# Digital-Defiance/node-fhe-accelerate

Hardware: AMD Instinct MI355X
Metric: NTTs/s at degree 16384 (batched, forward NTT + pointwise modmul) (higher is better)
Workload: dtype u64 (32-bit Shoup/Montgomery lanes for q<2^30); 1 GPU; C3: N=16384 forward NTT + modmul, batch 65536 per GPU, q=132120577; n=16384, batch_per_gpu=65536, global_batch=65536, q=132120577, parallelism=batch-sharded x1, no data-path collective

## Files before the change

node-fhe-accelerate_amd/csrc/fhe_gpu.cpp:

```cpp
#include <hip/hip_runtime.h>

#include <algorithm>
#include <cstdlib>
#include <cstdio>
#include <cstring>
#include <mutex>
#include <thread>
#include <string>
#include <vector>

#include "../../include/fhe_gpu.h"
#include "fhe_internal.hpp"
#include "keygen.hpp"
#include "build_id.h"

using u64 = uint64_t;
using u32 = uint32_t;
using u128 = unsigned __int128;

namespace {

thread_local std::string g_err;

int fail(int code, const std::string &msg) {
// ... 816 lines not shown
        c->inv_n = ref_mod_inverse(n, q);
    }
    c->fwd_tw.resize(n);
    c->inv_tw.resize(n);
    c->fwd_tw[0] = c->inv_tw[0] = 1;
    for (u32 i = 1; i < n; ++i) {
        c->fwd_tw[i] = mulmod(c->fwd_tw[i - 1], psi, q);
        c->inv_tw[i] = mulmod(c->inv_tw[i - 1], c->psi_inv, q);
    }
    DeviceGuard g(device);
    int rc = c->word == 32 ? build_tables<u32>(c, c->plan.a32) : build_tables<u64>(c, c->plan.a64);
    if (rc == FHE_OK && c->wide) rc = build_wide_tables(c);
    if (rc == FHE_OK && (int)logn > FHE_NS::kMaxFusedLogN) {
        c->plan.big_chunk = ((size_t)1 << 25) >> logn;
        for (auto &sp : c->plan.big_scratch) {
            hipError_t e = hipMalloc((void **)&sp, c->plan.big_chunk * n * sizeof(u64));
            if (e != hipSuccess) { rc = hip_fail(e, "hipMalloc(big-N scratch)"); break; }
        }
    }
    if (rc == FHE_OK) {
        hipError_t e = hipStreamCreateWithFlags(&c->own_stream, hipStreamNonBlocking);
        if (e != hipSuccess) rc = hip_fail(e, "hipStreamCreate");
    }
    if (rc == FHE_OK) {
        const char *kv = std::getenv("FHE_POOL_KEEP_MB");
        const uint64_t keep_mb = kv ? std::strtoull(kv, nullptr, 10) : 8192;
        hipMemPool_t pool = nullptr;
        if (keep_mb && hipDeviceGetDefaultMemPool(&pool, device) == hipSuccess && pool) {
            uint64_t keep = keep_mb << 20;
            (void)hipMemPoolSetAttribute(pool, hipMemPoolAttrReleaseThreshold, &keep);
        }
        (void)hipGetLastError();
    }
    if (rc != FHE_OK) {
        free_tables(c);
        delete c;
        return rc;
    }
    c->stream = c->own_stream;
    c->plan.logn = logn;
    c->plan.word = c->word;
    {
        int cus = 0;
        if (hipDeviceGetAttribute(&cus, hipDeviceAttributeMultiprocessorCount, device) != hipSuccess || cus <= 0) cus = 256;
        (void)hipGetLastError();
        c->plan.cus = cus;
    }
    c->plan.wide = c->wide;
    c->plan.lazy = c->word == 32 && (u128)(4 + 2 * logn) * q <= ((u128)1 << 32);
    {
        const char *u = std::getenv("FHE_UNIT_TW");
        c->plan.compat = c->mode == FHE_MODE_COMPAT && !(u && u[0] == '0');
    }
    c->plan.stream = c->stream;
    c->plan.big_sync = &c->big_sync;
    *out = c;
    return FHE_OK;
}

int fhe_ctx_create_multi(uint32_t n, uint64_t q, int mode, const int *devices, int ndev, fhe_ctx **out) {
    if (!out) return fail(FHE_ERR_INVALID_ARG, "null out");
    *out = nullptr;
    if (!devices || ndev < 1) return fail(FHE_ERR_INVALID_ARG, "at least one device required");
    fhe_ctx *m = new fhe_ctx();
    for (int i = 0; i < ndev; ++i) {
        fhe_ctx *s = nullptr;
        const int rc = fhe_ctx_create(n, q, mode, devices[i], &s);
        if (rc != FHE_OK) {
            const std::string msg = g_err;
            fhe_ctx_destroy(m);
            return fail(rc, msg);
        }
        m->subs.push_back(s);
    }
    const fhe_ctx *s0 = m->subs[0];
    m->n = s0->n; m->logn = s0->logn; m->q = s0->q; m->psi = s0->psi; m->psi_inv = s0->psi_inv;
    m->inv_n = s0->inv_n; m->mode = s0->mode; m->device = s0->device; m->word = s0->word;
    m->fwd_tw = s0->fwd_tw; m->inv_tw = s0->inv_tw;
    m->stream = s0->stream;
    *out = m;
    return FHE_OK;
}

int fhe_ctx_device_count(const fhe_ctx *c, int *ndev) {
    if (int rc = check_ctx(c)) return rc;
    if (!ndev) return fail(FHE_ERR_INVALID_ARG, "null out");
    *ndev = c->multi() ? (int)c->subs.size() : 1;
    return FHE_OK;
}

int fhe_ctx_sub(const fhe_ctx *c, int i, fhe_ctx **out) {
    if (int rc = check_ctx(c)) return rc;
    if (!out) return fail(FHE_ERR_INVALID_ARG, "null out");
    const int nd = c->multi() ? (int)c->subs.size() : 1;
    if (i < 0 || i >= nd) return fail(FHE_ERR_INVALID_ARG, "device index out of range");
    *out = c->multi() ? c->subs[i] : const_cast<fhe_ctx *>(c);
    return FHE_OK;
}

void fhe_ctx_destroy(fhe_ctx *c) {
    if (!c) return;
    if (c->multi()) {
        for (auto it = c->subs.rbegin(); it != c->subs.rend(); ++it) fhe_ctx_destroy(*it);
        delete c;
        return;
    }
// ... 2291 lines not shown
```

node-fhe-accelerate_amd/csrc/fhe_internal.hpp:

```cpp
#pragma once
#include <hip/hip_runtime.h>
#include <stddef.h>
#include <stdint.h>

#include <mutex>

#include "ntt_core.hpp"

namespace FHE_NS {

struct BigSync {
    std::mutex mu;
    hipEvent_t done = nullptr;
    hipStream_t last = nullptr;
};

struct WideArgs {
    const uint64_t *twf, *twi;
    uint64_t q, qinv, mu;
    uint64_t r2;
    uint64_t ninv_m;
    uint64_t ninv_r2;
};

struct Plan {
    uint32_t logn;
    int word;
    int wide;
    int lazy;
    int compat;
    int cus;
    hipStream_t stream;
    uint64_t *big_scratch[2];
    size_t big_chunk;
    BigSync *big_sync;
    NttArgs<uint32_t> a32;
    NttArgs<uint64_t> a64;
    WideArgs wa;
};

constexpr int kMinLogN = 2;
constexpr int kMaxFusedLogN = 14;
constexpr int kMaxLogN = 16;

hipError_t launch_fwd(const Plan &p, const uint64_t *in, uint64_t *out, size_t batch, int epi);
hipError_t launch_inv(const Plan &p, const uint64_t *in, uint64_t *out, size_t batch);
hipError_t launch_fwd_mul(const Plan &p, const uint64_t *a, const uint64_t *w, uint64_t *out, size_t batch);
hipError_t launch_polymul(const Plan &p, const uint64_t *a, const uint64_t *b, uint64_t *c, size_t batch);
hipError_t launch_fwd_limbs(const Plan &p, const void *tab, int limbs, const uint64_t *in, uint64_t *out,
                            size_t batch);
hipError_t launch_inv_limbs(const Plan &p, const void *tab, int limbs, const uint64_t *a, const uint64_t *b,
                            uint64_t *c, size_t batch);
hipError_t launch_wide(const Plan &p, int op, const uint64_t *a, const uint64_t *b, uint64_t *c, size_t batch);
hipError_t launch_big(const Plan &p, int op, const uint64_t *a, const uint64_t *b, uint64_t *c, size_t batch);
hipError_t launch_extprod(const Plan &p, int k1, int level, int base_log, const uint64_t *glwe,
                          const uint64_t *ggsw, uint64_t *out, size_t batch);
bool extprod_acc_supported(const Plan &p, int k1, int level, int base_log);
hipError_t launch_extprod_acc(const Plan &p, int level, int base_log, const uint64_t *glwe, const uint64_t *ggsw,
                              uint64_t *out, size_t batch);

hipError_t launch_relin(const Plan &p, int level, int base_log, const uint64_t *ct3, const uint64_t *rlk,
                        uint64_t *out, size_t batch);
hipError_t launch_cmux_rotate(const Plan &p, int k1, int level, int base_log, const uint64_t *acc_in,
                              const uint64_t *ggsw, uint64_t *acc_out, size_t batch, const uint64_t *lwe_a,
                              uint32_t lwe_dim, uint32_t step, uint64_t lwe_q);
bool br_persist_supported(const Plan &p, int k1);
struct BrPairOpts {
    uint64_t timeout_ticks;
    bool coop;
    unsigned long long *repairs;
    bool multi;
};
bool br_pair_supported(const Plan &p, int k1, size_t batch);
int br_multi_members(const Plan &p, int level, size_t batch);
size_t br_pair_scratch_bytes(const Plan &p, size_t batch, int level, bool multi);
hipError_t launch_br_pair(const Plan &p, int level, int base_log, uint64_t *acc, const uint64_t *bsk,
                          const uint64_t *lwe_a, const uint64_t *lwe_b, uint32_t lwe_dim, uint64_t lwe_q, size_t batch,
                          void *scratch, const BrPairOpts &o);
hipError_t launch_br_persist(const Plan &p, int k1, int level, int base_log, uint64_t *acc, const uint64_t *bsk,
                             const uint64_t *lwe_a, const uint64_t *lwe_b, uint32_t lwe_dim, uint64_t lwe_q,
                             size_t batch);
hipError_t launch_cmux(const Plan &p, int k1, int level, int base_log, const uint64_t *ggsw, const uint64_t *ct0,
                       const uint64_t *ct1, uint64_t *out, size_t batch);
hipError_t launch_ct_mul(const Plan &p, const uint64_t *x, const uint64_t *y, uint64_t *out, size_t batch);
// ... 110 lines not shown
```

node-fhe-accelerate_amd/csrc/ntt_core.hpp:

```cpp
#pragma once
#include "fhe_arith.hpp"

namespace FHE_NS {

constexpr int kPadA[17] = {0, 0, 0, 0, 0, 3, 3, 3, 4, 5, 5, 6, 7, 8, 5, 5, 0};
constexpr int kPadB[17] = {0, 0, 0, 0, 0, 0, 0, 0, 0, 0, 0, 0, 0, 0, 10, 10, 0};

constexpr int gk(int logn, int loge) { return logn | (loge << 8); }
constexpr int gk_logn(int k) { return k & 0xff; }
constexpr int gk_loge(int k) { return ((k >> 8) & 0xf) ? ((k >> 8) & 0xf) : ((k & 0xff) < 4 ? (k & 0xff) : 4); }
constexpr int gk_sparse(int k, int sel) { return k | (sel << 12); }
constexpr int gk_sp(int k) { return (k >> 12) & 3; }
constexpr int gk_compat(int k) { return k | (1 << 14); }
constexpr bool gk_cp(int k) { return (k >> 14) & 1; }

constexpr int pad_a(int L, int E) {
    return E == 5 ? 0 : (L == 10 && E == 3) ? 5 : (L == 10 && E == 2) ? 4 : kPadA[L];
}
constexpr int pad_b(int L, int E) {
    return E == 5 ? L - 5 : (L == 10 && E == 3) ? 6 : (L == 10 && E == 2) ? 5 : kPadB[L];
}
template <int K>
__host__ __device__ constexpr uint32_t pad_idx(uint32_t i) {
    constexpr int L = gk_logn(K);
// ... 286 lines not shown
}

struct NoHook {
    __device__ void operator()() const {}
};

template <int LOGN, int PASS, int K, int LOOK, bool LAZY, typename W>
__device__ __forceinline__ void fwd_stages(uint32_t tau, W (&v)[Geo<LOGN>::E], Tw<W> (&t)[PassTw<LOGN, PASS>::COUNT],
                                           const Tw<W> *__restrict__ tw, const Arith<W> &ar) {
    constexpr int R = PassTw<LOGN, PASS>::R;
    if constexpr (K < R) {
        if constexpr (K + LOOK < R) load_tw<LOGN, PASS, W, K + LOOK, K + LOOK + 1>(tau, tw, t);
        fwd_stage<LOGN, PASS, K, LAZY>(v, t, ar);
        __builtin_amdgcn_sched_barrier(0);
        fwd_stages<LOGN, PASS, K + 1, LOOK, LAZY>(tau, v, t, tw, ar);
    }
}
template <int LOGN, int PASS, int K, int LOOK, bool FOLD, typename W>
__device__ __forceinline__ void inv_stages(uint32_t tau, W (&v)[Geo<LOGN>::E], Tw<W> (&t)[PassTw<LOGN, PASS>::COUNT],
                                           const Tw<W> *__restrict__ tw, const Arith<W> &ar, Scale<W> scale) {
    if constexpr (K >= 0) {
        if constexpr (K - LOOK >= 0) load_tw<LOGN, PASS, W, K - LOOK, K - LOOK + 1>(tau, tw, t);
        inv_stage<LOGN, PASS, K, FOLD>(v, t, ar, scale);
        __builtin_amdgcn_sched_barrier(0);
        inv_stages<LOGN, PASS, K - 1, LOOK, FOLD>(tau, v, t, tw, ar, scale);
    }
}
template <int LOGN>
constexpr bool staged_tw() { return Geo<LOGN>::LOGE >= 5; }

#ifndef FHE_STREAM_DEPTH
#define FHE_STREAM_DEPTH 4
#endif
template <int LOGN, typename W>
constexpr bool stream_tw() { return sizeof(W) == 8 && Geo<LOGN>::LOGE == 5; }
#ifndef FHE_STREAM_TW2
#define FHE_STREAM_TW2 0
#endif
template <int LOGN, typename W>
constexpr bool stream_tw2() { return FHE_STREAM_TW2 && Geo<LOGN>::LOGE == 5; }
constexpr int kStreamDepth = FHE_STREAM_DEPTH;

struct SItem { int k, u, tl; };
__host__ __device__ constexpr SItem stream_item(int R, int NU, bool inv, int i) {
    for (int s = 0; s < R; ++s) {
        const int k = inv ? R - 1 - s : s;
        if (i < NU << k) return SItem{k, i >> k, i & ((1 << k) - 1)};
        i -= NU << k;
    }
    return SItem{0, 0, 0};
}

template <int LOGN, int PASS, typename W>
__device__ __forceinline__ Tw<W> tw_one(uint32_t tau, const Tw<W> *__restrict__ tw, SItem it) {
    using G = Geo<LOGN>;
    constexpr int S = G::S(PASS);
    if constexpr (PASS == 0) {
        typedef const __attribute__((address_space(4))) W cw_t;
        const cw_t *cp = (const cw_t *)(const void *)tw;
        const uint32_t idx = (1u << it.k) + uint32_t(it.tl);
        return Tw<W>{cp[2 * idx], cp[2 * idx + 1]};
    } else {
        static_assert(G::P == 1, "streamed twiddles: one polynomial per workgroup");
        constexpr uint32_t m = (1u << S) - 1;
        const uint32_t cst = (1u << (S + it.k)) + ((uint32_t(it.u) << G::LOGT) & m) + (uint32_t(it.tl) << S);
        return bload_tw<W>(brsrc(tw), (tau & m) * (uint32_t)sizeof(Tw<W>), cst * (uint32_t)sizeof(Tw<W>));
    }
}

template <int LOGN, int PASS, bool INV, bool SKIP0, int I, typename W>
__device__ __forceinline__ void stream_load(uint32_t tau, const Tw<W> *__restrict__ tw,
                                            Tw<W> (&b)[PassTw<LOGN, PASS>::COUNT]) {
    using P = PassTw<LOGN, PASS>;
    if constexpr (I < P::COUNT) {
        constexpr SItem it = stream_item(P::R, P::NU, INV, I);
        if constexpr (!(SKIP0 && it.k == 0))
            b[I] = tw_one<LOGN, PASS>(tau, tw, it);
    }
}
template <int LOGN, int PASS, bool INV, bool SKIP0, int I = 0, typename W>
__device__ __forceinline__ void stream_begin(uint32_t tau, const Tw<W> *__restrict__ tw,
                                             Tw<W> (&b)[PassTw<LOGN, PASS>::COUNT]) {
    if constexpr (I < kStreamDepth) {
        stream_load<LOGN, PASS, INV, SKIP0, I>(tau, tw, b);
        stream_begin<LOGN, PASS, INV, SKIP0, I + 1>(tau, tw, b);
    }
}
template <int LOGN, int PASS, bool LAZY, bool RS, bool D2 = false, int I = 0, typename W>
__device__ __forceinline__ void fwd_pass_stream(uint32_t tau, W (&v)[Geo<LOGN>::E], Tw<W> (&b)[PassTw<LOGN, PASS>::COUNT],
                                                const Tw<W> *__restrict__ tw, const Arith<W> &ar, Scale<W> rmod = Scale<W>{},
                                                W (*v2)[Geo<LOGN>::E] = nullptr) {
    using P = PassTw<LOGN, PASS>;
    constexpr int R = P::R;
    constexpr bool SK = RS && PASS == 0;
    if constexpr (I < P::COUNT) {
        stream_load<LOGN, PASS, false, SK, I + kStreamDepth>(tau, tw, b);
        constexpr SItem it = stream_item(R, P::NU, false, I);
        constexpr int k = it.k;
#pragma unroll
        for (int h = 0; h < (D2 ? 2 : 1); ++h) {
            W (&x)[Geo<LOGN>::E] = h ? *v2 : v;
#pragma unroll
            for (int tt = 0; tt < (1 << R); ++tt) {
                if ((tt & (1 << k)) || (tt & ((1 << k) - 1)) != it.tl) continue;
                const int e = tt + (it.u << R), e2 = e + (1 << k);
                if constexpr (SK && k == 0) ar.template ct_rscale<gk_sp(LOGN)>(x[e], x[e2], rmod);
                else if constexpr (LAZY) ar.template ct_lazy<gk_sp(LOGN)>(x[e], x[e2], b[I]);
                else ar.template ct<gk_sp(LOGN)>(x[e], x[e2], b[I]);
            }
        }
        __builtin_amdgcn_sched_barrier(0);
        fwd_pass_stream<LOGN, PASS, LAZY, RS, D2, I + 1>(tau, v, b, tw, ar, rmod, v2);
    }
}
template <int LOGN, int PASS, bool FOLD, bool D2 = false, int I = 0, typename W>
__device__ __forceinline__ void inv_pass_stream(uint32_t tau, W (&v)[Geo<LOGN>::E], Tw<W> (&b)[PassTw<LOGN, PASS>::COUNT],
                                                const Tw<W> *__restrict__ tw, const Arith<W> &ar, Scale<W> scale,
                                                W (*v2)[Geo<LOGN>::E] = nullptr) {
    using P = PassTw<LOGN, PASS>;
    constexpr int R = P::R;
    constexpr bool SK = FOLD && PASS == 0;
    if constexpr (I < P::COUNT) {
        stream_load<LOGN, PASS, true, SK, I + kStreamDepth>(tau, tw, b);
        constexpr SItem it = stream_item(R, P::NU, true, I);
        constexpr int k = it.k;
#pragma unroll
        for (int h = 0; h < (D2 ? 2 : 1); ++h) {
            W (&x)[Geo<LOGN>::E] = h ? *v2 : v;
#pragma unroll
            for (int tt = 0; tt < (1 << R); ++tt) {
                if ((tt & (1 << k)) || (tt & ((1 << k) - 1)) != it.tl) continue;
                const int e = tt + (it.u << R), e2 = e + (1 << k);
                if constexpr (SK && k == 0) ar.template gs_scaled<gk_sp(LOGN)>(x[e], x[e2], scale);
                else ar.template gs<gk_sp(LOGN)>(x[e], x[e2], b[I]);
            }
        }
        __builtin_amdgcn_sched_barrier(0);
        inv_pass_stream<LOGN, PASS, FOLD, D2, I + 1>(tau, v, b, tw, ar, scale, v2);
    }
}

template <int LOGN, int PASS, bool LAZY, int PF, typename W, typename H = NoHook>
__device__ __forceinline__ void fwd_rest(W *lds, W (&v)[Geo<LOGN>::E], uint32_t tau, const Tw<W> *__restrict__ tw,
                                         const Arith<W> &ar, H &&hook = NoHook{}) {
    using G = Geo<LOGN>;
    if constexpr (PASS < G::NP) {
        Tw<W> t[PassTw<LOGN, PASS>::COUNT];
        if constexpr (stream_tw<LOGN, W>()) {
            stream_begin<LOGN, PASS, false, false>(tau, tw, t);
            exchange<LOGN, PASS - 1, PASS>(lds, v, tau);
            if constexpr (PASS == G::NP - 1) hook();
            fwd_pass_stream<LOGN, PASS, LAZY, false>(tau, v, t, tw, ar);
            fwd_rest<LOGN, PASS + 1, LAZY, PF>(lds, v, tau, tw, ar, hook);
            return;
        }
        load_tw<LOGN, PASS, W, 0, PF>(tau, tw, t);
        exchange<LOGN, PASS - 1, PASS>(lds, v, tau);
        if constexpr (staged_tw<LOGN>()) {
            if constexpr (PASS == G::NP - 1) hook();
            fwd_stages<LOGN, PASS, 0, PF, LAZY>(tau, v, t, tw, ar);
        } else {
            load_tw<LOGN, PASS, W, PF, 8>(tau, tw, t);
            if constexpr (PASS == G::NP - 1) hook();
            fwd_pass<LOGN, PASS, LAZY>(v, t, ar);
        }
        fwd_rest<LOGN, PASS + 1, LAZY, PF>(lds, v, tau, tw, ar, hook);
    }
}

template <int LOGN, int PASS, int K, int LOOK, bool LAZY, typename W>
__device__ __forceinline__ void fwd_stages2(uint32_t tau, W (&v)[Geo<LOGN>::E], W (&v2)[Geo<LOGN>::E],
                                            Tw<W> (&t)[PassTw<LOGN, PASS>::COUNT], const Tw<W> *__restrict__ tw,
                                            const Arith<W> &ar) {
    constexpr int R = PassTw<LOGN, PASS>::R;
    if constexpr (K < R) {
        if constexpr (K + LOOK < R) load_tw<LOGN, PASS, W, K + LOOK, K + LOOK + 1>(tau, tw, t);
        fwd_stage<LOGN, PASS, K, LAZY>(v, t, ar);
        fwd_stage<LOGN, PASS, K, LAZY>(v2, t, ar);
        __builtin_amdgcn_sched_barrier(0);
        fwd_stages2<LOGN, PASS, K + 1, LOOK, LAZY>(tau, v, v2, t, tw, ar);
    }
}
template <int LOGN, int PASS, bool LAZY, int PF, typename W>
__device__ __forceinline__ void fwd_rest2(W *lds, W (&v)[Geo<LOGN>::E], W (&v2)[Geo<LOGN>::E], uint32_t tau,
                                          const Tw<W> *__restrict__ tw, const Arith<W> &ar) {
    using G = Geo<LOGN>;
    if constexpr (PASS < G::NP) {
        Tw<W> t[PassTw<LOGN, PASS>::COUNT];
        if constexpr (stream_tw2<LOGN, W>()) {
            stream_begin<LOGN, PASS, false, false>(tau, tw, t);
            exchange<LOGN, PASS - 1, PASS>(lds, v, tau);
            __syncthreads();
            exchange<LOGN, PASS - 1, PASS>(lds, v2, tau);
            fwd_pass_stream<LOGN, PASS, LAZY, false, true>(tau, v, t, tw, ar, Scale<W>{}, &v2);
            fwd_rest2<LOGN, PASS + 1, LAZY, PF>(lds, v, v2, tau, tw, ar);
            return;
        }
        load_tw<LOGN, PASS, W, 0, PF>(tau, tw, t);
        exchange<LOGN, PASS - 1, PASS>(lds, v, tau);
        __syncthreads();
        exchange<LOGN, PASS - 1, PASS>(lds, v2, tau);
        fwd_stages2<LOGN, PASS, 0, PF, LAZY>(tau, v, v2, t, tw, ar);
        fwd_rest2<LOGN, PASS + 1, LAZY, PF>(lds, v, v2, tau, tw, ar);
    }
}

template <int LOGN, int PASS, bool FOLD, int PF, typename W>
__device__ __forceinline__ void inv_rest(W *lds, W (&v)[Geo<LOGN>::E], uint32_t tau, const Tw<W> *__restrict__ tw,
                                         const Arith<W> &ar, Scale<W> scale) {
    if constexpr (PASS >= 0) {
        Tw<W> t[PassTw<LOGN, PASS>::COUNT];
        if constexpr (stream_tw<LOGN, W>()) {
            stream_begin<LOGN, PASS, true, FOLD && PASS == 0>(tau, tw, t);
            exchange<LOGN, PASS + 1, PASS>(lds, v, tau);
            inv_pass_stream<LOGN, PASS, FOLD>(tau, v, t, tw, ar, scale);
            inv_rest<LOGN, PASS - 1, FOLD, PF>(lds, v, tau, tw, ar, scale);
            return;
        }
        constexpr int R = PassTw<LOGN, PASS>::R;
        constexpr int KS = R - PF < 0 ? 0 : R - PF;
        load_tw<LOGN, PASS, W, KS, 8>(tau, tw, t);
        exchange<LOGN, PASS + 1, PASS>(lds, v, tau);
        if constexpr (staged_tw<LOGN>()) {
            inv_stages<LOGN, PASS, R - 1, R - KS, FOLD>(tau, v, t, tw, ar, scale);
        } else {
            load_tw<LOGN, PASS, W, 0, KS>(tau, tw, t);
            inv_pass<LOGN, PASS, FOLD>(v, t, ar, scale);
        }
        inv_rest<LOGN, PASS - 1, FOLD, PF>(lds, v, tau, tw, ar, scale);
    }
}

template <typename W>
struct NttArgs {
    const Tw<W> *twf;
    const Tw<W> *twi;
    Arith<W> ar;
    uint64_t q64, mu64;
    Scale<W> ninv;
    Scale<W> ninv_r;
    Scale<W> rs;
    Tw<W> rmod;
    Tw<W> one;
};

template <bool LAZY, typename W>
__device__ __forceinline__ W fwd_to_2q(W x, const NttArgs<W> &A) {
    if constexpr (LAZY) return A.ar.shoup(x, A.one);
    else return A.ar.red2q(x);
}
template <bool LAZY, typename W>
__device__ __forceinline__ W fwd_to_canon(W x, const NttArgs<W> &A) {
    return A.ar.red1q(fwd_to_2q<LAZY>(x, A));
}

template <typename W>
// ... 37 lines not shown
    uint64_t raw[E];
#pragma unroll
    for (int t = 0; t < E; ++t) raw[t] = addr_of(t);
    uint32_t bad = 0;
#pragma unroll
    for (int t = 0; t < E; ++t) {
        bad |= uint32_t(raw[t] >= lim) << t;
        v[t] = W(raw[t]);
    }
    if (__builtin_expect(bad != 0, 0)) {
#pragma unroll
        for (int t = 0; t < E; ++t)
            if ((bad >> t) & 1) v[t] = W(red(addr_of(t)));
    }
}
template <int E, typename W, typename F>
__device__ __forceinline__ void load_coeffs(W (&v)[E], uint64_t lim, uint64_t q, uint64_t mu, F &&addr_of) {
    uint64_t raw[E];
#pragma unroll
    for (int t = 0; t < E; ++t) raw[t] = addr_of(t);
    coeffs_from_raw<E>(v, raw, lim, Mod64Red{q, mu});
}

constexpr int kLoadInflight = 1;
constexpr int kPoly2Chunk = 8;
template <int E, int CH, int IN, typename W, typename RD, typename F>
__device__ __forceinline__ void load_coeffs_chunked(W (&v)[E], uint64_t lim, RD &&red, F &&addr_of) {
    constexpr int NC = E / CH;
    uint64_t raw[E];
#pragma unroll
    for (int c = 0; c < IN && c < NC; ++c)
#pragma unroll
        for (int t = c * CH; t < c * CH + CH; ++t) raw[t] = addr_of(t);
#pragma unroll
    for (int c = 0; c < NC; ++c) {
        if (c + IN < NC) {
#pragma unroll
            for (int t = (c + IN) * CH; t < (c + IN) * CH + CH; ++t) raw[t] = addr_of(t);
        }
        __builtin_amdgcn_sched_barrier(0);
        uint32_t bad = 0;
#pragma unroll
        for (int t = c * CH; t < c * CH + CH; ++t) {
            bad |= uint32_t(raw[t] >= lim) << (t - c * CH);
            v[t] = W(raw[t]);
        }
        if (__builtin_expect(bad != 0, 0)) {
#pragma unroll
            for (int t = c * CH; t < c * CH + CH; ++t)
                if ((bad >> (t - c * CH)) & 1) v[t] = W(red(addr_of(t)));
        }
        __builtin_amdgcn_sched_barrier(0);
    }
}

template <int LOGN, bool LAZY, int PF = kPfSingle, bool RS = false, typename W, typename H = NoHook>
__device__ __forceinline__ void fwd_poly(W *lds, W (&v)[Geo<LOGN>::E], uint32_t tau, const uint64_t *__restrict__ src,
                                         bool valid, const NttArgs<W> &A, uint32_t sh = 0, H &&hook = NoHook{}, uint64_t (*pre)[Geo<LOGN>::E] = nullptr) {
    using G = Geo<LOGN>;
    constexpr bool ST = stream_tw<LOGN, W>();
    const Tw<W> *const twf = opaque_tw(A.twf);
    Tw<W> t0[PassTw<LOGN, 0>::COUNT];
    if constexpr (!ST) load_tw<LOGN, 0>(tau, twf, t0);
    const uint64_t lim = RS ? (uint64_t)(W)~W(0) : (uint64_t)(A.ar.q2 * 2);
    if (pre) {
        coeffs_from_raw<G::E>(v, *pre, lim, SlowRed<W>{A});
    } else if constexpr (G::P == 1) {
        const auto r = brsrc(src);
        const uint32_t vo = (tau << sh) * 8u;
        auto at = [&](int t) -> uint64_t { return bload(r, vo, ((cbrv(t, G::LOGE) * G::T) << sh) * 8u); };
        if constexpr (G::LOGE == 5) load_coeffs_chunked<G::E, 8, kLoadInflight>(v, lim, SlowRed<W>{A}, at);
        else load_coeffs_r<G::E>(v, lim, SlowRed<W>{A}, at);
    } else {
        load_coeffs_r<G::E>(v, lim, SlowRed<W>{A}, [&](int t) -> uint64_t {
            return valid ? __builtin_nontemporal_load(src + ((tau + cbrv(t, G::LOGE) * G::T) << sh)) : 0;
        });
    }
    if constexpr (ST) {
        stream_begin<LOGN, 0, false, RS>(tau, twf, t0);
        fwd_pass_stream<LOGN, 0, LAZY, RS>(tau, v, t0, twf, A.ar, A.rs);
    } else {
        fwd_pass<LOGN, 0, LAZY, W, RS>(v, t0, A.ar, A.rs);
    }
    fwd_rest<LOGN, 1, LAZY, PF>(lds, v, tau, twf, A.ar, hook);
}

template <int LOGN, bool LAZY, int PF, typename W>
__device__ __forceinline__ void fwd_poly2(W *lds, W (&v)[Geo<LOGN>::E], W (&v2)[Geo<LOGN>::E], uint32_t tau,
                                          const uint64_t *__restrict__ src, const uint64_t *__restrict__ src2,
                                          const NttArgs<W> &A) {
    using G = Geo<LOGN>;
    static_assert(G::P == 1, "dual transform: one polynomial pair per workgroup");
    constexpr bool ST = stream_tw2<LOGN, W>();
    const Tw<W> *const twf = opaque_tw(A.twf);
    Tw<W> t0[PassTw<LOGN, 0>::COUNT];
    if constexpr (!ST) load_tw<LOGN, 0>(tau, twf, t0);
    const uint64_t lim = (uint64_t)(A.ar.q2 * 2);
    const uint32_t vo = tau * 8u;
    {
        const auto r = brsrc(src);
        load_coeffs_chunked<G::E, kPoly2Chunk, kLoadInflight>(v, lim, SlowRed<W>{A}, [&](int t) -> uint64_t {
            return bload(r, vo, cbrv(t, G::LOGE) * G::T * 8u);
        });
    }
    {
        const auto r = brsrc(src2);
// ... 177 lines not shown
```

node-fhe-accelerate_amd/csrc/ntt_inv.hip:

```cpp
#ifndef FHE_SPLIT_X64
#define FHE_SPLIT_X64 1
#endif
#ifndef FHE_U64_NOVCC
#define FHE_U64_NOVCC 1
#endif
#ifndef FHE_MULHI64
#define FHE_MULHI64 4
#endif
#include "fhe_internal.hpp"

namespace FHE_NS {

template <int LOGN, typename W>
__device__ __forceinline__ void ntt_inv_body(const uint64_t *__restrict__ in, uint64_t *__restrict__ out, size_t batch,
                                             const NttArgs<W> &A) {
    using G = Geo<LOGN>;
    __shared__ W lds_all[G::P * lds_elems<LOGN, W>()];
    const uint32_t tau = threadIdx.x & (G::T - 1), pl = wg_poly<G>();
    const size_t poly = (size_t)blockIdx.x * G::P + pl;
    const bool valid = poly < batch;
    W *lds = lds_all + pl * lds_elems<LOGN, W>();
    if (G::P == 1 && !valid) return;
    W v[G::E];
    const uint64_t *src = in + poly * G::N;
// ... 72 lines not shown
        if constexpr (STASH == 0) va[e] = x;
        else st[gi] = x;
    }
    if constexpr (G::NP > 1) __syncthreads();
    uint32_t tb = tau;
    if constexpr (sizeof(W) == 8) asm volatile("" : "+v"(tb));
    if constexpr (PRE)
        fwd_poly<LOGN, LAZY, kPfPolymul>(lds, v, tb, b + poly * G::N, valid, A, 0, NoHook{},
                                               reinterpret_cast<uint64_t(*)[G::E]>(rb));
    else
        fwd_poly<LOGN, LAZY, kPfPolymul>(lds, v, tb, b + poly * G::N, valid, A);
#pragma unroll
    for (int e = 0; e < G::E; ++e) {
        const uint32_t gi = gidx<LOGN, G::NP - 1>(tb, e);
        W x;
        if constexpr (STASH == 0) x = va[e];
        else x = st[gi];
        v[e] = A.ar.mont(x, v[e]);
    }
    if constexpr (G::NP > 1) __syncthreads();
    uint32_t ti = tau;
    if constexpr (sizeof(W) == 8) asm volatile("" : "+v"(ti));
    inv_poly_from_regs<LOGN, kPfPolymul>(lds, v, ti, crow, valid, A, A.ninv_r);
}
template <int LOGN, typename W, bool LAZY>
__global__ void __launch_bounds__(Geo<LOGN>::THREADS, 1)
k_polymul(const uint64_t *__restrict__ a, const uint64_t *__restrict__ b, uint64_t *c, size_t batch,
          NttArgs<W> A) {
    polymul_body<LOGN, W, LAZY>(a, b, c, batch, A);
}
template <int LOGN, typename W, bool LAZY>
__global__ void __launch_bounds__(Geo<LOGN>::THREADS)
k_polymul_limbs(const uint64_t *__restrict__ a, const uint64_t *__restrict__ b, uint64_t *c, size_t batch,
                const NttArgs<W> *__restrict__ tab) {
    const size_t o = (size_t)blockIdx.y * batch * Geo<LOGN>::N;
    const NttArgs<W> A = tab[blockIdx.y];
    polymul_body<LOGN, W, LAZY>(a + o, b + o, c + o, batch, A);
}

template <int LOGN, typename W, bool LAZY>
__device__ __forceinline__ void polymul2_one(W *lds, uint32_t tau, const uint64_t *__restrict__ a,
                                             const uint64_t *__restrict__ b, uint64_t *c, size_t poly,
                                             const NttArgs<W> &A) {
    using G = Geo<LOGN>;
    W v[G::E], vb[G::E];
    fwd_poly2<LOGN, LAZY, polymul2_pf<LOGN, W>()>(lds, v, vb, tau, a + poly * G::N, b + poly * G::N, A);
#pragma unroll
    for (int e = 0; e < G::E; ++e) v[e] = A.ar.mont(fwd_to_canon<LAZY>(v[e], A), vb[e]);
    __syncthreads();
    inv_poly_from_regs<LOGN, polymul2_pf<LOGN, W>()>(lds, v, tau, c + poly * G::N, true, A, A.ninv_r);
}

template <int LOGN, typename W>
constexpr int polymul2_occ() {
    constexpr int o = Geo<LOGN>::template occ_waves<W>();
    return (Geo<LOGN>::LOGE == 4 && (sizeof(W) == 4 || gk_logn(LOGN) < 14) && o > 4) ? 4 : o;
}
template <int LOGN, typename W, bool LAZY>
__global__ void __launch_bounds__(Geo<LOGN>::THREADS, (polymul2_occ<LOGN, W>()))
k_polymul2(const uint64_t *__restrict__ a, const uint64_t *__restrict__ b, uint64_t *c, size_t batch,
           NttArgs<W> A) {
    using G = Geo<LOGN>;
    static_assert(G::P == 1, "one polynomial pair per workgroup");
    __shared__ W lds[lds_elems<LOGN, W>()];
    const uint32_t tau = threadIdx.x;
    const size_t poly = blockIdx.x;
    if (poly >= batch) return;
    polymul2_one<LOGN, W, LAZY>(lds, tau, a, b, c, poly, A);
}
template <int LOGN, typename W, bool LAZY>
__global__ void __launch_bounds__(Geo<LOGN>::THREADS)
k_polymul2_limbs(const uint64_t *__restrict__ a, const uint64_t *__restrict__ b, uint64_t *c, size_t batch,
                 const NttArgs<W> *__restrict__ tab) {
    __shared__ W lds[lds_elems<LOGN, W>()];
    const size_t poly = blockIdx.x;
    if (poly >= batch) return;
    const size_t o = (size_t)blockIdx.y * batch * Geo<LOGN>::N;
    const NttArgs<W> A = tab[blockIdx.y];
    polymul2_one<LOGN, W, LAZY>(lds, threadIdx.x, a + o, b + o, c + o, poly, A);
}

template <int LOGN, typename W>
static hipError_t inv_one(const Plan &p, const NttArgs<W> &A, hipStream_t s, const uint64_t *a, const uint64_t *b,
                          uint64_t *c, size_t batch, const NttArgs<W> *tab = nullptr, int limbs = 1) {
    auto go = [&](auto K, auto KL, size_t blocks, int threads, auto... args) -> hipError_t {
        if (tab)
            hipLaunchKernelGGL(KL, dim3((unsigned)blocks, (unsigned)limbs), dim3(threads), 0, s, args..., tab);
        else
            hipLaunchKernelGGL(K, dim3((unsigned)blocks), dim3(threads), 0, s, args..., A);
        return hipGetLastError();
    };
    bool lazy = false;
    if constexpr (sizeof(W) == 4) lazy = p.lazy;
    constexpr int PK = polymul_key<LOGN, W>();
    using GP = Geo<PK>;
    size_t pblocks = (batch + GP::P - 1) / GP::P;
    if constexpr (polymul_dual<PK, W>()) {
        if (b) {
            if constexpr (sizeof(W) == 4) {
                if (lazy)
                    return go(k_polymul2<PK, W, true>, k_polymul2_limbs<PK, W, true>, pblocks, GP::THREADS, a, b, c,
                              batch);
            }
            if constexpr (sizeof(W) == 8) {
                if (!tab && A.ar.sp == 1 && p.compat)
                    return go(k_polymul2<gk_compat(gk_sparse(PK, 1)), W, false>, k_polymul2_limbs<PK, W, false>,
                              pblocks, GP::THREADS, a, b, c, batch);
                if (!tab && A.ar.sp == 1)
                    return go(k_polymul2<gk_sparse(PK, 1), W, false>, k_polymul2_limbs<PK, W, false>, pblocks,
                              GP::THREADS, a, b, c, batch);
                if (!tab && A.ar.sp == 2)
                    return go(k_polymul2<gk_sparse(PK, 2), W, false>, k_polymul2_limbs<PK, W, false>, pblocks,
                              GP::THREADS, a, b, c, batch);
                if (!tab && p.compat)
                    return go(k_polymul2<gk_compat(PK), W, false>, k_polymul2_limbs<PK, W, false>, pblocks,
                              GP::THREADS, a, b, c, batch);
            }
            return go(k_polymul2<PK, W, false>, k_polymul2_limbs<PK, W, false>, pblocks, GP::THREADS, a, b, c, batch);
        }
    } else {
        if (b && lazy) {
            if constexpr (sizeof(W) == 4)
                return go(k_polymul<PK, W, true>, k_polymul_limbs<PK, W, true>, pblocks, GP::THREADS, a, b, c, batch);
            return hipErrorInvalidValue;
        } else if (b) {
            return go(k_polymul<PK, W, false>, k_polymul_limbs<PK, W, false>, pblocks, GP::THREADS, a, b, c, batch);
        }
    }
    using GI = Geo<LOGN>;
    const size_t iblocks = (batch + GI::P - 1) / GI::P;
    return go(k_ntt_inv<LOGN, W>, k_ntt_inv_limbs<LOGN, W>, iblocks, GI::THREADS, a, c, batch);
}

template <typename W>
static hipError_t inv_dispatch(const Plan &p, const NttArgs<W> &A, const uint64_t *a, const uint64_t *b,
                               uint64_t *c, size_t batch) {
    switch (p.logn) {
#define FHE_CASE(L) \
    case L: return inv_one<L, W>(p, A, p.stream, a, b, c, batch);
        FHE_CASE(2) FHE_CASE(3) FHE_CASE(4) FHE_CASE(5) FHE_CASE(6) FHE_CASE(7) FHE_CASE(8)
        FHE_CASE(9) FHE_CASE(10) FHE_CASE(11) FHE_CASE(12) FHE_CASE(13) FHE_CASE(14)
#undef FHE_CASE
    default: return hipErrorInvalidValue;
    }
}

static hipError_t inv_any(const Plan &p, const uint64_t *a, const uint64_t *b, uint64_t *c, size_t batch) {
    if (batch == 0) return hipSuccess;
    if (p.word == 32)
        return inv_dispatch<uint32_t>(p, p.a32, a, b, c, batch);
    return inv_dispatch<uint64_t>(p, p.a64, a, b, c, batch);
// ... 41 lines not shown
```

Measured before the change: 14.80 million NTTs/s.

## Add streamed polymul kernel with LDS-cached pass-1 twiddles and chunked input overlap

For 32-bit words at N=16384 with a 32-element-per-thread geometry, k_polymul2 gains a specialised path. It copies the pass-1 forward and inverse twiddle tables into LDS once per workgroup. It streams the second operand's loads in chunks that overlap the first polynomial's pass-0 butterflies, and reads arguments from the kernarg segment to reduce SGPR/VGPR pressure. An env knob (FHE_POLYMUL_STREAM=0) falls back to the old kernel. The extra LDS holds the twiddle tables and is capped so two workgroups still fit per CU, at the cost of a per-block table fill and a more complex schedule.

```diff
diff --git a/node-fhe-accelerate_amd/csrc/fhe_gpu.cpp b/node-fhe-accelerate_amd/csrc/fhe_gpu.cpp
--- a/node-fhe-accelerate_amd/csrc/fhe_gpu.cpp
+++ b/node-fhe-accelerate_amd/csrc/fhe_gpu.cpp
@@ -892,6 +892,10 @@
         const char *u = std::getenv("FHE_UNIT_TW");
         c->plan.compat = c->mode == FHE_MODE_COMPAT && !(u && u[0] == '0');
     }
+    {
+        const char *u = std::getenv("FHE_POLYMUL_STREAM");
+        c->plan.pm_stream = !(u && u[0] == '0');
+    }
     c->plan.stream = c->stream;
     c->plan.big_sync = &c->big_sync;
     *out = c;
diff --git a/node-fhe-accelerate_amd/csrc/fhe_internal.hpp b/node-fhe-accelerate_amd/csrc/fhe_internal.hpp
--- a/node-fhe-accelerate_amd/csrc/fhe_internal.hpp
+++ b/node-fhe-accelerate_amd/csrc/fhe_internal.hpp
@@ -30,6 +30,7 @@
     int lazy;
     int compat;
     int cus;
+    int pm_stream;
     hipStream_t stream;
     uint64_t *big_scratch[2];
     size_t big_chunk;
diff --git a/node-fhe-accelerate_amd/csrc/ntt_core.hpp b/node-fhe-accelerate_amd/csrc/ntt_core.hpp
--- a/node-fhe-accelerate_amd/csrc/ntt_core.hpp
+++ b/node-fhe-accelerate_amd/csrc/ntt_core.hpp
@@ -362,10 +362,23 @@
 }
 
 template <int LOGN, int PASS, typename W>
+__device__ __forceinline__ const Tw<W> *lds_tw_lane(const Tw<W> *tab, uint32_t tau) {
+    typedef const __attribute__((address_space(3))) Tw<W> lds_tw;
+    uint32_t a = (uint32_t)(size_t)(lds_tw *)(tab + (tau & ((1u << Geo<LOGN>::S(PASS)) - 1)));
+    asm volatile("" : "+v"(a));
+    return reinterpret_cast<const Tw<W> *>((size_t)a);
+}
+template <int LOGN, int PASS, bool LT = false, typename W>
 __device__ __forceinline__ Tw<W> tw_one(uint32_t tau, const Tw<W> *__restrict__ tw, SItem it) {
     using G = Geo<LOGN>;
     constexpr int S = G::S(PASS);
-    if constexpr (PASS == 0) {
+    if constexpr (LT) {
+        static_assert(PASS > 0 && sizeof(Tw<W>) == 8 && G::P == 1, "LDS twiddles: 32-bit words, a lane-indexed pass");
+        constexpr uint32_t m = (1u << S) - 1;
+        const uint32_t cst = (1u << (S + it.k)) + ((uint32_t(it.u) << G::LOGT) & m) + (uint32_t(it.tl) << S);
+        typedef const __attribute__((address_space(3))) uint64_t lds_u64;
+        return __builtin_bit_cast(Tw<W>, ((lds_u64 *)(size_t)(uint32_t)(size_t)tw)[cst - (1u << S)]);
+    } else if constexpr (PASS == 0) {
         typedef const __attribute__((address_space(4))) W cw_t;
         const cw_t *cp = (const cw_t *)(const void *)tw;
         const uint32_t idx = (1u << it.k) + uint32_t(it.tl);
@@ -378,25 +391,25 @@
     }
 }
 
-template <int LOGN, int PASS, bool INV, bool SKIP0, int I, typename W>
+template <int LOGN, int PASS, bool INV, bool SKIP0, int I, bool LT = false, typename W>
 __device__ __forceinline__ void stream_load(uint32_t tau, const Tw<W> *__restrict__ tw,
                                             Tw<W> (&b)[PassTw<LOGN, PASS>::COUNT]) {
     using P = PassTw<LOGN, PASS>;
     if constexpr (I < P::COUNT) {
         constexpr SItem it = stream_item(P::R, P::NU, INV, I);
         if constexpr (!(SKIP0 && it.k == 0))
-            b[I] = tw_one<LOGN, PASS>(tau, tw, it);
-    }
-}
-template <int LOGN, int PASS, bool INV, bool SKIP0, int I = 0, typename W>
+            b[I] = tw_one<LOGN, PASS, LT>(tau, tw, it);
+    }
+}
+template <int LOGN, int PASS, bool INV, bool SKIP0, int I = 0, bool LT = false, typename W>
 __device__ __forceinline__ void stream_begin(uint32_t tau, const Tw<W> *__restrict__ tw,
                                              Tw<W> (&b)[PassTw<LOGN, PASS>::COUNT]) {
     if constexpr (I < kStreamDepth) {
-        stream_load<LOGN, PASS, INV, SKIP0, I>(tau, tw, b);
-        stream_begin<LOGN, PASS, INV, SKIP0, I + 1>(tau, tw, b);
-    }
-}
-template <int LOGN, int PASS, bool LAZY, bool RS, bool D2 = false, int I = 0, typename W>
+        stream_load<LOGN, PASS, INV, SKIP0, I, LT>(tau, tw, b);
+        stream_begin<LOGN, PASS, INV, SKIP0, I + 1, LT>(tau, tw, b);
+    }
+}
+template <int LOGN, int PASS, bool LAZY, bool RS, bool D2 = false, int I = 0, bool LT = false, typename W>
 __device__ __forceinline__ void fwd_pass_stream(uint32_t tau, W (&v)[Geo<LOGN>::E], Tw<W> (&b)[PassTw<LOGN, PASS>::COUNT],
                                                 const Tw<W> *__restrict__ tw, const Arith<W> &ar, Scale<W> rmod = Scale<W>{},
                                                 W (*v2)[Geo<LOGN>::E] = nullptr) {
@@ -404,7 +417,7 @@
     constexpr int R = P::R;
     constexpr bool SK = RS && PASS == 0;
     if constexpr (I < P::COUNT) {
-        stream_load<LOGN, PASS, false, SK, I + kStreamDepth>(tau, tw, b);
+        stream_load<LOGN, PASS, false, SK, I + kStreamDepth, LT>(tau, tw, b);
         constexpr SItem it = stream_item(R, P::NU, false, I);
         constexpr int k = it.k;
 #pragma unroll
@@ -420,18 +433,18 @@
             }
         }
         __builtin_amdgcn_sched_barrier(0);
-        fwd_pass_stream<LOGN, PASS, LAZY, RS, D2, I + 1>(tau, v, b, tw, ar, rmod, v2);
-    }
-}
-template <int LOGN, int PASS, bool FOLD, bool D2 = false, int I = 0, typename W>
+        fwd_pass_stream<LOGN, PASS, LAZY, RS, D2, I + 1, LT>(tau, v, b, tw, ar, rmod, v2);
+    }
+}
+template <int LOGN, int PASS, bool FOLD, bool D2 = false, int I = 0, bool LT = false, int IE = -1, typename W>
 __device__ __forceinline__ void inv_pass_stream(uint32_t tau, W (&v)[Geo<LOGN>::E], Tw<W> (&b)[PassTw<LOGN, PASS>::COUNT],
                                                 const Tw<W> *__restrict__ tw, const Arith<W> &ar, Scale<W> scale,
                                                 W (*v2)[Geo<LOGN>::E] = nullptr) {
     using P = PassTw<LOGN, PASS>;
     constexpr int R = P::R;
     constexpr bool SK = FOLD && PASS == 0;
-    if constexpr (I < P::COUNT) {
-        stream_load<LOGN, PASS, true, SK, I + kStreamDepth>(tau, tw, b);
+    if constexpr (I < (IE < 0 ? P::COUNT : IE)) {
+        stream_load<LOGN, PASS, true, SK, I + kStreamDepth, LT>(tau, tw, b);
         constexpr SItem it = stream_item(R, P::NU, true, I);
         constexpr int k = it.k;
 #pragma unroll
@@ -446,7 +459,7 @@
             }
         }
         __builtin_amdgcn_sched_barrier(0);
-        inv_pass_stream<LOGN, PASS, FOLD, D2, I + 1>(tau, v, b, tw, ar, scale, v2);
+        inv_pass_stream<LOGN, PASS, FOLD, D2, I + 1, LT, IE>(tau, v, b, tw, ar, scale, v2);
     }
 }
 
@@ -491,12 +504,22 @@
         fwd_stages2<LOGN, PASS, K + 1, LOOK, LAZY>(tau, v, v2, t, tw, ar);
     }
 }
-template <int LOGN, int PASS, bool LAZY, int PF, typename W>
+template <int LOGN, int PASS, bool LAZY, int PF, bool LT = false, typename W>
 __device__ __forceinline__ void fwd_rest2(W *lds, W (&v)[Geo<LOGN>::E], W (&v2)[Geo<LOGN>::E], uint32_t tau,
-                                          const Tw<W> *__restrict__ tw, const Arith<W> &ar) {
+                                          const Tw<W> *__restrict__ tw, const Arith<W> &ar,
+                                          const Tw<W> *__restrict__ ltw = nullptr) {
     using G = Geo<LOGN>;
     if constexpr (PASS < G::NP) {
         Tw<W> t[PassTw<LOGN, PASS>::COUNT];
+        if constexpr (LT && PASS == 1) {
+            stream_begin<LOGN, PASS, false, false, 0, true>(tau, ltw, t);
+            exchange<LOGN, PASS - 1, PASS>(lds, v, tau);
+            __syncthreads();
+            exchange<LOGN, PASS - 1, PASS>(lds, v2, tau);
+            fwd_pass_stream<LOGN, PASS, LAZY, false, true, 0, true>(tau, v, t, ltw, ar, Scale<W>{}, &v2);
+            fwd_rest2<LOGN, PASS + 1, LAZY, PF, LT>(lds, v, v2, tau, tw, ar, ltw);
+            return;
+        }
         if constexpr (stream_tw2<LOGN, W>()) {
             stream_begin<LOGN, PASS, false, false>(tau, tw, t);
             exchange<LOGN, PASS - 1, PASS>(lds, v, tau);
@@ -511,7 +534,7 @@
         __syncthreads();
         exchange<LOGN, PASS - 1, PASS>(lds, v2, tau);
         fwd_stages2<LOGN, PASS, 0, PF, LAZY>(tau, v, v2, t, tw, ar);
-        fwd_rest2<LOGN, PASS + 1, LAZY, PF>(lds, v, v2, tau, tw, ar);
+        fwd_rest2<LOGN, PASS + 1, LAZY, PF, LT>(lds, v, v2, tau, tw, ar, ltw);
     }
 }
 
@@ -655,6 +678,36 @@
         }
         __builtin_amdgcn_sched_barrier(0);
     }
+}
+
+template <int LOGN, int C>
+__device__ __forceinline__ void chunk_issue(uint64_t (&raw)[kPoly2Chunk], __amdgpu_buffer_rsrc_t r, uint32_t vo) {
+    using G = Geo<LOGN>;
+    __builtin_amdgcn_sched_barrier(0);
+#pragma unroll
+    for (int t = 0; t < kPoly2Chunk; ++t) raw[t] = bload(r, vo, cbrv(C * kPoly2Chunk + t, G::LOGE) * G::T * 8u);
+    __builtin_amdgcn_sched_barrier(0);
+}
+template <int LOGN, int C, int EV, typename W, typename RD>
+__device__ __forceinline__ void chunk_narrow(W (&v)[EV], uint64_t (&raw)[kPoly2Chunk], uint64_t lim, RD &&red,
+                                             __amdgpu_buffer_rsrc_t r, uint32_t vo) {
+    using G = Geo<LOGN>;
+    static_assert((C + 1) * kPoly2Chunk <= EV, "chunk within the destination");
+    __builtin_amdgcn_sched_barrier(0);
+    uint32_t bad = 0;
+#pragma unroll
+    for (int t = 0; t < kPoly2Chunk; ++t) {
+        bad |= uint32_t(raw[t] >= lim) << t;
+        if constexpr (sizeof(W) == 4) asm("v_mov_b32 %0, %1" : "=v"(v[C * kPoly2Chunk + t]) : "v"((uint32_t)raw[t]));
+        else v[C * kPoly2Chunk + t] = W(raw[t]);
+    }
+    if (__builtin_expect(bad != 0, 0)) {
+#pragma unroll
+        for (int t = 0; t < kPoly2Chunk; ++t)
+            if ((bad >> t) & 1)
+                v[C * kPoly2Chunk + t] = W(red(bload(r, vo, cbrv(C * kPoly2Chunk + t, G::LOGE) * G::T * 8u)));
+    }
+    __builtin_amdgcn_sched_barrier(0);
 }
 
 template <int LOGN, bool LAZY, int PF = kPfSingle, bool RS = false, typename W, typename H = NoHook>
diff --git a/node-fhe-accelerate_amd/csrc/ntt_inv.hip b/node-fhe-accelerate_amd/csrc/ntt_inv.hip
--- a/node-fhe-accelerate_amd/csrc/ntt_inv.hip
+++ b/node-fhe-accelerate_amd/csrc/ntt_inv.hip
@@ -148,6 +148,166 @@
 }
 
 template <int LOGN, typename W>
+constexpr bool polymul_stream() { return sizeof(W) == 4 && LOGN == gk(14, 5); }
+template <int LOGN, typename W>
+struct StreamLds {
+    using G = Geo<LOGN>;
+    static constexpr int LO = 1 << G::S(1), CNT = (1 << G::S(2)) - LO;
+    static constexpr int BASE = (lds_elems<LOGN, W>() + 1) & ~1;
+    static constexpr int WORDS = BASE + 2 * CNT * (int)(sizeof(Tw<W>) / sizeof(W));
+    static_assert(WORDS * (int)sizeof(W) <= 80 * 1024, "two workgroups per CU");
+};
+__device__ __forceinline__ uint32_t per_phase(uint32_t tau) {
+    asm volatile("" : "+v"(tau));
+    return tau;
+}
+template <typename W>
+struct PolymulArgs {
+    const uint64_t *a, *b;
+    uint64_t *c;
+    size_t batch;
+    NttArgs<W> A;
+};
+template <typename W>
+__device__ __forceinline__ const __attribute__((address_space(4))) PolymulArgs<W> *polymul_kargs() {
+    typedef const __attribute__((address_space(4))) PolymulArgs<W> kargs_t;
+    kargs_t *k = (kargs_t *)__builtin_amdgcn_kernarg_segment_ptr();
+    asm volatile("" : "+s"(k));
+    return k;
+}
+template <typename W>
+__device__ __forceinline__ NttArgs<W> kargs_ntt(const __attribute__((address_space(4))) PolymulArgs<W> *k) {
+#if defined(__HIP_DEVICE_COMPILE__)
+    return k->A;
+#else
+    (void)k;
+    return NttArgs<W>{};
+#endif
+}
+template <typename W>
+struct SlowRedK {
+    __device__ __forceinline__ uint64_t operator()(uint64_t x) const {
+        const NttArgs<W> A = kargs_ntt<W>(polymul_kargs<W>());
+        return SlowRed<W>{A}(x);
+    }
+};
+template <int LOGN, typename W>
+__device__ __forceinline__ void stream_inv_tail(W *lds, W (&v)[Geo<LOGN>::E],
+                                                uint32_t tau0, const Tw<W> *lti, const Tw<W> *twi,
+                                                __amdgpu_buffer_rsrc_t rc,
+                                                const NttArgs<W> &A) {
+    using G = Geo<LOGN>;
+    const Scale<W> sc = A.ninv_r;
+    tau0 = per_phase(tau0);
+    uint32_t tau = tau0, vo = tau * 8u;
+    {
+        Tw<W> t[PassTw<LOGN, 1>::COUNT];
+        const Tw<W> *const lane = lds_tw_lane<LOGN, 1>(lti, tau);
+        stream_begin<LOGN, 1, true, false, 0, true>(tau, lane, t);
+        inv_pass_stream<LOGN, 1, true, false, 0, true, 16>(tau, v, t, lane, A.ar, sc);
+        inv_pass_stream<LOGN, 1, true, false, 16, true, 24>(tau, v, t, lane, A.ar, sc);
+        inv_pass_stream<LOGN, 1, true, false, 24, true, 28>(tau, v, t, lane, A.ar, sc);
+        inv_pass_stream<LOGN, 1, true, false, 28, true, 30>(tau, v, t, lane, A.ar, sc);
+        inv_pass_stream<LOGN, 1, true, false, 30, true>(tau, v, t, lane, A.ar, sc);
+    }
+    exchange<LOGN, 1, 0>(lds, v, tau);
+    tau0 = per_phase(tau0);
+    tau = tau0, vo = tau * 8u;
+    {
+        Tw<W> t[PassTw<LOGN, 0>::COUNT];
+        load_tw<LOGN, 0>(tau, twi, t);
+        inv_pass<LOGN, 0, true>(v, t, A.ar, sc);
+    }
+#pragma unroll
+    for (int t = 0; t < G::E; ++t) bstore(rc, vo, cbrv(t, G::LOGE) * G::T * 8u, (uint64_t)A.ar.red1q(v[t]));
+}
+template <int LOGN, typename W, bool LAZY>
+__device__ __forceinline__ void polymul2_stream(W *lds, uint32_t tau0) {
+    using G = Geo<LOGN>;
+    using SL = StreamLds<LOGN, W>;
+    static_assert(kPoly2Chunk * 4 == G::E && G::NP == 3, "four chunks per polynomial, three passes");
+    constexpr int PF = polymul2_pf<LOGN, W>();
+    uint64_t *tab = reinterpret_cast<uint64_t *>(lds + SL::BASE);
+    const Tw<W> *ltf = reinterpret_cast<const Tw<W> *>(tab), *lti = ltf + SL::CNT;
+    {
+        const auto *const k = polymul_kargs<W>();
+        const uint64_t *gf = reinterpret_cast<const uint64_t *>(k->A.twf) + SL::LO;
+        const uint64_t *gi = reinterpret_cast<const uint64_t *>(k->A.twi) + SL::LO;
+        for (uint32_t i = tau0; i < 2u * SL::CNT; i += G::T) tab[i] = i < (uint32_t)SL::CNT ? gf[i] : gi[i - SL::CNT];
+    }
+    __syncthreads();
+    const uint32_t poly = blockIdx.x;
+    W v[G::E], vb[G::E];
+    {
+        const auto *const k = polymul_kargs<W>();
+        const NttArgs<W> A = kargs_ntt<W>(k);
+        const uint64_t lim = (uint64_t)(A.ar.q2 * 2);
+        const SlowRedK<W> red{};
+        const uint32_t vo = tau0 * 8u;
+        const auto ra = brsrc(k->a + (size_t)poly * G::N);
+        uint64_t raw[kPoly2Chunk];
+        chunk_issue<LOGN, 0>(raw, ra, vo);
+        chunk_narrow<LOGN, 0>(vb, raw, lim, red, ra, vo);
+        chunk_issue<LOGN, 1>(raw, ra, vo);
+        chunk_narrow<LOGN, 1>(vb, raw, lim, red, ra, vo);
+        chunk_issue<LOGN, 2>(raw, ra, vo);
+        chunk_narrow<LOGN, 2>(vb, raw, lim, red, ra, vo);
+        chunk_issue<LOGN, 3>(raw, ra, vo);
+        chunk_narrow<LOGN, 3>(vb, raw, lim, red, ra, vo);
+    }
+    {
+        tau0 = per_phase(tau0);
+        uint32_t tau = tau0;
+        const auto *k = polymul_kargs<W>();
+        {
+            const NttArgs<W> A = kargs_ntt<W>(k);
+            const uint64_t lim = (uint64_t)(A.ar.q2 * 2);
+            const SlowRed<W> red{A};
+            const uint32_t vo = tau * 8u;
+            const auto rb = brsrc(k->b + (size_t)poly * G::N);
+            const Tw<W> *const twf = A.twf;
+            Tw<W> t0[PassTw<LOGN, 0>::COUNT];
+            load_tw<LOGN, 0>(tau, twf, t0);
+            uint64_t r0[kPoly2Chunk], r1[kPoly2Chunk];
+            chunk_issue<LOGN, 0>(r0, rb, vo);
+            chunk_issue<LOGN, 1>(r1, rb, vo);
+            fwd_stage<LOGN, 0, 0, LAZY>(vb, t0, A.ar);
+            fwd_stage<LOGN, 0, 1, LAZY>(vb, t0, A.ar);
+            fwd_stage<LOGN, 0, 2, LAZY>(vb, t0, A.ar);
+            chunk_narrow<LOGN, 0>(v, r0, lim, red, rb, vo);
+            chunk_issue<LOGN, 2>(r0, rb, vo);
+            fwd_stage<LOGN, 0, 3, LAZY>(vb, t0, A.ar);
+            chunk_narrow<LOGN, 1>(v, r1, lim, red, rb, vo);
+            chunk_issue<LOGN, 3>(r1, rb, vo);
+            fwd_stage<LOGN, 0, 4, LAZY>(vb, t0, A.ar);
+            chunk_narrow<LOGN, 2>(v, r0, lim, red, rb, vo);
+            chunk_narrow<LOGN, 3>(v, r1, lim, red, rb, vo);
+            fwd_pass<LOGN, 0, LAZY, W>(v, t0, A.ar);
+            fwd_rest2<LOGN, 1, LAZY, PF, true>(lds, v, vb, tau, twf, A.ar, lds_tw_lane<LOGN, 1>(ltf, tau));
+        }
+        k = polymul_kargs<W>();
+        const NttArgs<W> A = kargs_ntt<W>(k);
+#pragma unroll
+        for (int e = 0; e < G::E; ++e) v[e] = A.ar.mont(fwd_to_canon<LAZY>(v[e], A), vb[e]);
+        __syncthreads();
+        tau0 = per_phase(tau0);
+        tau = tau0;
+        const Tw<W> *const twi = A.twi;
+        {
+            constexpr int R = PassTw<LOGN, 2>::R;
+            Tw<W> t[PassTw<LOGN, 2>::COUNT];
+            load_tw<LOGN, 2, W, R - 1, 8>(tau, twi, t);
+            inv_stages<LOGN, 2, R - 1, 1, true>(tau, v, t, twi, A.ar, A.ninv_r);
+        }
+        exchange<LOGN, 2, 1>(lds, v, tau);
+    }
+    const auto *const k = polymul_kargs<W>();
+    const auto rc = brsrc(k->c + (size_t)poly * G::N);
+    const NttArgs<W> A = kargs_ntt<W>(k);
+    stream_inv_tail<LOGN>(lds, v, tau0, lti, A.twi, rc, A);
+}
+
+template <int LOGN, typename W>
 constexpr int polymul2_occ() {
     constexpr int o = Geo<LOGN>::template occ_waves<W>();
     return (Geo<LOGN>::LOGE == 4 && (sizeof(W) == 4 || gk_logn(LOGN) < 14) && o > 4) ? 4 : o;
@@ -158,11 +318,28 @@
            NttArgs<W> A) {
     using G = Geo<LOGN>;
     static_assert(G::P == 1, "one polynomial pair per workgroup");
+    if constexpr (polymul_stream<LOGN, W>()) {
+        __shared__ __attribute__((aligned(8))) W lds[StreamLds<LOGN, W>::WORDS];
+        if (blockIdx.x >= batch) return;
+        static_assert(offsetof(PolymulArgs<W>, A) == 32 && alignof(NttArgs<W>) == 8, "k_polymul2's argument layout");
+        polymul2_stream<LOGN, W, LAZY>(lds, threadIdx.x);
+    } else {
+        __shared__ W lds[lds_elems<LOGN, W>()];
+        const uint32_t tau = threadIdx.x;
+        const size_t poly = blockIdx.x;
+        if (poly >= batch) return;
+        polymul2_one<LOGN, W, LAZY>(lds, tau, a, b, c, poly, A);
+    }
+}
+template <int LOGN, typename W, bool LAZY>
+__global__ void __launch_bounds__(Geo<LOGN>::THREADS, (polymul2_occ<LOGN, W>()))
+k_polymul2_pair(const uint64_t *__restrict__ a, const uint64_t *__restrict__ b, uint64_t *c, size_t batch,
+                NttArgs<W> A) {
+    static_assert(polymul_stream<LOGN, W>(), "elsewhere k_polymul2 is this kernel");
     __shared__ W lds[lds_elems<LOGN, W>()];
-    const uint32_t tau = threadIdx.x;
     const size_t poly = blockIdx.x;
     if (poly >= batch) return;
-    polymul2_one<LOGN, W, LAZY>(lds, tau, a, b, c, poly, A);
+    polymul2_one<LOGN, W, LAZY>(lds, threadIdx.x, a, b, c, poly, A);
 }
 template <int LOGN, typename W, bool LAZY>
 __global__ void __launch_bounds__(Geo<LOGN>::THREADS)
@@ -193,6 +370,13 @@
     size_t pblocks = (batch + GP::P - 1) / GP::P;
     if constexpr (polymul_dual<PK, W>()) {
         if (b) {
+            if constexpr (polymul_stream<PK, W>()) {
+                if (!tab) {
+                    if (!p.pm_stream && lazy)
+                        return go(k_polymul2_pair<PK, W, true>, k_polymul2_limbs<PK, W, true>, pblocks, GP::THREADS,
+                                  a, b, c, batch);
+                }
+            }
             if constexpr (sizeof(W) == 4) {
                 if (lazy)
                     return go(k_polymul2<PK, W, true>, k_polymul2_limbs<PK, W, true>, pblocks, GP::THREADS, a, b, c,
```

Measured after the change: 14.14 million NTTs/s. -4.5%, worse.
